# MGI-tech-bioinformatics/SuperPlus

Hardware: AMD Instinct MI355X
Metric: k-mers/s (DF createDict stage: trim + canonical k-mer count + solid filter + spectrum + adjacency) (higher is better)
Workload: dtype u64

## Files before the change

### superplus_amd/csrc/dfk.hip

```cpp
#include "../../include/dfk.h"
#include "dfk_kernels.h"

#include <algorithm>
#include <chrono>
#include <cstdarg>
#include <cstdio>
#include <cstdlib>
#include <cstring>
#include <atomic>
#include <fcntl.h>
#include <functional>
#include <new>
#include <string>
#include <sys/mman.h>
#include <sys/stat.h>
#include <unistd.h>
#include <condition_variable>
#include <memory>
#include <mutex>
#include <thread>
#include <vector>

using namespace dfk;

namespace {

thread_local std::string g_err;

int fail(int code, const char* fmt, ...)
{
    char buf[512];
    va_list ap; va_start(ap, fmt); vsnprintf(buf, sizeof buf, fmt, ap); va_end(ap);
    g_err = buf;
    return code;
}

#define HIP_TRY(expr) do { hipError_t e_ = (expr); if (e_ != hipSuccess) \
    return fail(DFK_E_HIP, "%s failed: %s (%s:%d)", #expr, hipGetErrorString(e_), __FILE__, __LINE__); } while (0)

template <class F> int guarded(F&& f)
{
    try { return f(); }
    catch (const std::bad_alloc&) { return fail(DFK_E_NOMEM, "out of host memory"); }
    catch (const std::exception& e) { return fail(DFK_E_HIP, "internal error: %s", e.what()); }
    catch (...) { return fail(DFK_E_HIP, "internal error"); }
}

struct DevBuf {
    void* p = nullptr; size_t bytes = 0;
    bool sub = false;
};

bool g_trace = getenv("DFK_TRACE") != nullptr;
#define TRACE(...) do { if (g_trace) { fprintf(stderr, "[dfk] " __VA_ARGS__); fputc('\n', stderr); fflush(stderr); } } while (0)
inline double wall_now() { return std::chrono::duration<double>(std::chrono::steady_clock::now().time_since_epoch()).count(); }

template <int K> struct CountCfg;
#ifndef DFK_LOG2S
#define DFK_LOG2S 11
#endif
#ifndef DFK_NWAVES
#define DFK_NWAVES 8
#endif
template <> struct CountCfg<40> { static constexpr int LOG2S = DFK_LOG2S, NWAVES = DFK_NWAVES; };
template <> struct CountCfg<48> { static constexpr int LOG2S = DFK_LOG2S, NWAVES = DFK_NWAVES; };
template <> struct CountCfg<60> { static constexpr int LOG2S = DFK_LOG2S, NWAVES = DFK_NWAVES; };

struct Inputs {
    const uint8_t* packed; uint64_t packed_bytes;
    const uint64_t* base_off; const uint32_t* read_len;
    const uint8_t* pq; uint64_t pq_bytes; const uint64_t* pq_off;
    const int32_t* bc; uint64_t n_reads;
};

}

struct dfk_ctx {
    dfk_config cfg{};
    int device = 0;
    hipStream_t stream = nullptr;
    hipStream_t stream2 = nullptr;
    hipDeviceProp_t prop{};
    uint64_t budget = 0, held = 0, peak = 0;
    struct Owned { void* p; uint64_t bytes, seq; };
    std::vector<Owned> owned;
    uint64_t alloc_seq = 0;
    bool have = false;
    uint64_t n_reads = 0;
    struct FileRange { const char* base; uint64_t bytes; int fd; uint64_t off; };
    std::vector<FileRange> file_ranges;
    DevBuf good_len;
    struct Part { DevBuf buf, pre; uint64_t n = 0; uint64_t blist = 0, n_blist = 0; bool listed = false; };
    bool want_blist = false;
    int pending_blist = -1;
    std::function<int()> after_count_launch;
    std::vector<Part> parts;
    uint64_t n_solid = 0, n_boundary = 0;
    unsigned seg_attempt = 0;
    double distinct_per_inst = 0.0;
    double plan_derate = 0.95;
    std::vector<int64_t> hist;
    std::vector<dfk_entry32> sorted, sorted_pre;
    bool sorted_ok = false, sorted_pre_ok = false;
    dfk_stats st{};
    bool shard_open = false, shard_use_bc = false;
    const void* sh_in[7] = {};
    uint64_t sh_packed_bytes = 0, sh_pq_bytes = 0, sh_n_reads = 0, sh_n_inst_local = 0;
    int64_t sh_read_id0 = 0;
    DevBuf shard_send[2];
    uint32_t shard_send_pass[2] = {~0u, ~0u};
    DevBuf shard_recv[2];
    unsigned shard_recv_seq = 0;
    uint64_t budget_taken = 0;
    void* sh_staged[6] = {};
    uint64_t sh_b0 = 0, sh_b1 = 0, sh_q0 = 0, sh_q1 = 0, sh_staged_reads = 0;
    DevBuf adj_keys, adj_src; uint64_t adj_n = 0;
    DevBuf set; uint64_t set_mask = 0;
    double t_upload_done = 0;
    uint32_t shard_world = 1, shard_log2_nb = 0;
    void* shard_state = nullptr;
    void (*shard_state_free)(void*) = nullptr;
    void* lane_pool = nullptr; void (*lane_pool_free)(void*) = nullptr;
    std::mutex lane_mu;
    void* graph_state = nullptr;
    void (*graph_state_free)(void*) = nullptr;
    unsigned int* d_resident = nullptr;
    unsigned int resident_target = 0;
    unsigned int last_wg_idle = 0;
    void* kept[6] = {};
    uint64_t kept_packed_bytes = 0, kept_pq_bytes = 0, kept_n_reads = 0, kept_budget = 0;

    struct Free { uint64_t off, bytes; };
    struct Chunk { char* p; uint64_t bytes; std::vector<Free> free_list; bool adopted = false; };
    std::vector<Chunk> chunks;
    uint64_t reserved = 0;

    uint64_t first_chunk_hint = 0;
    bool carve(Chunk& k, size_t bytes, DevBuf& b, bool long_lived)
    {
        if (!long_lived) {
            for (size_t i = k.free_list.size(); i-- > 0;)
                if (k.free_list[i].bytes >= bytes) {
                    k.free_list[i].bytes -= bytes;
                    b.p = k.p + k.free_list[i].off + k.free_list[i].bytes; b.bytes = bytes;
                    if (!k.free_list[i].bytes) k.free_list.erase(k.free_list.begin() + i);
                    return true;
                }
            return false;
        }
        for (size_t i = 0; i < k.free_list.size(); ++i)
            if (k.free_list[i].bytes >= bytes) {
                b.p = k.p + k.free_list[i].off; b.bytes = bytes;
                k.free_list[i].off += bytes; k.free_list[i].bytes -= bytes;
                if (!k.free_list[i].bytes) k.free_list.erase(k.free_list.begin() + i);
                return true;
            }
        return false;
    }
    void drop_empty_chunks()
    {
        for (size_t i = 0; i < chunks.size();)
            if (chunks[i].free_list.size() == 1 && chunks[i].free_list[0].bytes == chunks[i].bytes)
            { (void)hipFree(chunks[i].p); reserved -= chunks[i].bytes; chunks.erase(chunks.begin() + i); }
            else ++i;
    }
    struct PassBlock { DevBuf block; size_t used = 0; };
    PassBlock* sub = nullptr;
    int alloc(DevBuf& b, size_t bytes, const char* what, bool top = false)
    {
        bytes = bytes ? (bytes + 255) & ~(size_t)255 : 256;
        if (sub && !top && sub->used + bytes <= sub->block.bytes) {
            b.p = (char*)sub->block.p + sub->used; b.bytes = bytes; b.sub = true;
            sub->used += bytes;
            return 0;
        }
        if (held + bytes > budget)
            return fail(DFK_E_NOMEM, "HBM budget exceeded allocating %zu bytes for %s (held %llu, budget %llu)",
                        bytes, what, (unsigned long long)held, (unsigned long long)budget);
        bool ok = false;
        for (Chunk& k : chunks) if (carve(k, bytes, b, top)) { ok = true; break; }
        if (!ok) {
            uint64_t want = std::max<uint64_t>(2 * (uint64_t)bytes, 64ull << 20);
            if (chunks.empty()) want = std::max<uint64_t>(want, std::min<uint64_t>(first_chunk_hint, budget));
            if (reserved + want > budget) { drop_empty_chunks(); want = std::min<uint64_t>(want, budget > reserved ? budget - reserved : 0); }
            want &= ~(uint64_t)0xFFF;
            if (want < bytes) {
                if (g_trace) {
                    for (const Chunk& k : chunks) for (const Free& f : k.free_list) fprintf(stderr, "[dfk]   free %.2f GB at %.2f GB\n", f.bytes / 1e9, f.off / 1e9);
                    for (const Owned& o : owned) if (o.bytes >= (1ull << 28)) fprintf(stderr, "[dfk]   held %.2f GB at %.2f GB (#%llu)\n", o.bytes / 1e9, ((char*)o.p - chunks[0].p) / 1e9, (unsigned long long)o.seq);
                }
                return fail(DFK_E_NOMEM, "HBM budget exhausted by fragmentation allocating %zu bytes for %s", bytes, what);
            }
            void* p = nullptr;
            hipError_t e = hipMalloc(&p, want);
            if (e != hipSuccess && want > bytes) { (void)hipGetLastError(); want = bytes; e = hipMalloc(&p, want); }
            if (e != hipSuccess) return fail(DFK_E_NOMEM, "hipMalloc(%llu) for %s: %s", (unsigned long long)want, what, hipGetErrorString(e));
            chunks.push_back(Chunk{(char*)p, want, {Free{0, want}}});
            reserved += want;
            TRACE("new device chunk %p, %.2f GB (reserved %.2f of %.2f GB)", p, want / 1e9, (reserved) / 1e9, budget / 1e9);
            carve(chunks.back(), bytes, b, top);
        }
        held += bytes; peak = std::max(peak, held);
        owned.push_back(Owned{b.p, (uint64_t)bytes, ++alloc_seq});
        if (bytes >= (1ull << 30)) TRACE("alloc %-28s %8.2f GB at %p (%s), held %.2f GB", what, bytes / 1e9, b.p, top ? "top" : "bottom", held / 1e9);
        return 0;
    }
    uint64_t largest_allocatable() const
    {
        uint64_t best = budget > reserved ? (budget - reserved) & ~(uint64_t)0xFFF : 0;
        for (const Chunk& k : chunks) for (const Free& f : k.free_list) best = std::max<uint64_t>(best, f.bytes);
        return std::min<uint64_t>(best, budget > held ? budget - held : 0);
    }
    void release(DevBuf& b)
    {
        if (!b.p) return;
        if (b.sub) { b = DevBuf{}; return; }
        auto it = std::find_if(owned.begin(), owned.end(), [&](const Owned& o) { return o.p == b.p; });
        if (it != owned.end()) owned.erase(it);
        for (Chunk& k : chunks)
// ... 1955 lines not shown
```

### superplus_amd/csrc/dfk_kernels.h

```cpp
#pragma once
#include <type_traits>
#include "dfk_device.h"

namespace dfk {

template <int K>
__global__ void __launch_bounds__(256)
k_trim(const uint8_t* __restrict__ pq, const uint64_t* __restrict__ pq_off, uint64_t pq_nbytes,
       const uint64_t* __restrict__ base_off, uint64_t packed_bytes, const uint32_t* __restrict__ read_len,
       uint64_t n_reads, uint32_t min_qual, uint32_t* __restrict__ good_len,
       unsigned long long* __restrict__ n_inst, unsigned int* __restrict__ bad,
       unsigned long long* __restrict__ sum_good)
{
    unsigned long long mine = 0, good = 0;
    bool any_bad = false;
    for (uint64_t r = (uint64_t)blockIdx.x * blockDim.x + threadIdx.x; r < n_reads; r += (uint64_t)gridDim.x * blockDim.x) {
        uint32_t gl = 0;
        uint64_t p = pq_off[r], end = pq_off[r + 1];
        uint32_t idx = 0, run = 0;
        const uint64_t b0 = base_off[r], b1 = base_off[r + 1];
        bool ok = p <= end && end <= pq_nbytes && b0 <= b1 && b1 <= packed_bytes && b1 - b0 >= ((uint64_t)read_len[r] + 3) / 4;
        if (!ok) end = p;
        while (p < end) {
            uint32_t nQs = pq[p];
            if (!nQs) break;
            if (p + 3 > end) { ok = false; break; }
            uint32_t hdr = pq[p + 1] | ((uint32_t)pq[p + 2] << 8);
            uint32_t nBits = hdr & 7u, minQ = (hdr >> 3) & 63u;
            uint64_t blk = ((uint64_t)nQs * nBits + 24) >> 3;
            if (p + blk > end) { ok = false; break; }
            if (nBits == 0) {
                if (minQ >= min_qual) { run += nQs; if (run >= (uint32_t)K) gl = idx + nQs; }
                else run = 0;
                idx += nQs;
            } else {
                uint64_t bit = 8 * (p + 1) + 9;
                const uint32_t fmask = (1u << nBits) - 1u;
                for (uint32_t left = nQs; left;) {
                    const uint64_t by = bit >> 3;
                    const uint32_t sh = (uint32_t)(bit & 7);
                    uint64_t w = 0;
                    if (by + 8 <= pq_nbytes) __builtin_memcpy(&w, pq + by, 8);
                    else for (uint32_t k = 0; k < 8 && by + k < pq_nbytes; ++k) w |= (uint64_t)pq[by + k] << (8 * k);
                    w >>= sh;
                    const uint32_t n = min(left, (64u - sh) / nBits);
                    for (uint32_t i = 0; i < n; ++i, w >>= nBits) {
                        const uint32_t q = minQ + ((uint32_t)w & fmask);
                        if (q < min_qual) run = 0;
                        else if (++run >= (uint32_t)K) gl = idx + 1;
                        ++idx;
                    }
                    bit += (uint64_t)n * nBits; left -= n;
                }
            }
            p += blk;
        }
        uint32_t rl = read_len[r];
        if (!ok || idx != rl) { any_bad = true; gl = 0; }
        if (gl > rl) gl = rl;
        good_len[r] = gl;
        good += gl;
        if (gl >= (uint32_t)K + 1) mine += gl - K + 1;
    }
    __shared__ unsigned long long sh[2][4];
    __shared__ unsigned int sh_bad;
    if (threadIdx.x == 0) sh_bad = 0;
    __syncthreads();
#pragma unroll
    for (int d = 32; d > 0; d >>= 1) { mine += __shfl_down(mine, d, 64); good += __shfl_down(good, d, 64); }
    if ((threadIdx.x & 63) == 0) { sh[0][threadIdx.x >> 6] = mine; sh[1][threadIdx.x >> 6] = good; }
    if (any_bad) atomicOr(&sh_bad, 1u);
    __syncthreads();
    if (threadIdx.x == 0) {
        unsigned long long a0 = sh[0][0] + sh[0][1] + sh[0][2] + sh[0][3], a1 = sh[1][0] + sh[1][1] + sh[1][2] + sh[1][3];
        if (a0) atomicAdd(n_inst, a0);
        if (a1) atomicAdd(sum_good, a1);
        if (sh_bad) atomicOr(bad, 1u);
    }
}

struct PartParams {
    uint32_t M;
    uint32_t W;
    uint32_t log2_nb;
    uint32_t log2_world;
    int64_t  read_id0;
    uint32_t sub_lo;
    uint32_t sub_n;
    uint32_t class_mask;
};

constexpr uint32_t SWEEP_CLASSES = 32;
__host__ __device__ inline uint32_t sweep_class_of(uint32_t local_bucket, uint32_t log2_local)
{ return log2_local > 5 ? local_bucket >> (log2_local - 5) : local_bucket; }
__host__ __device__ inline uint32_t sweep_class_mask(uint32_t sub_lo, uint32_t sub_n, uint32_t log2_local)
{
    if (sub_n == 0) return 0u;
    const uint32_t a = sweep_class_of(sub_lo, log2_local), b = sweep_class_of(sub_lo + sub_n - 1, log2_local);
    const uint32_t upto_b = b >= 31 ? 0xFFFFFFFFu : ((1u << (b + 1)) - 1u);
    return upto_b & ~((1u << a) - 1u);
}

constexpr int PART_THREADS = 128;
constexpr int PART_RING = 2;
constexpr int SUMMARY_RUNS = 10;
constexpr uint32_t SUMMARY_OVERFLOW = 15;

__device__ __forceinline__ uint32_t pass_local(uint32_t bucket, const PartParams& pp)
{
    const uint32_t ls = pp.log2_nb - pp.log2_world;
    const uint32_t d = (bucket & ((1u << ls) - 1u)) - pp.sub_lo;
    return d < pp.sub_n ? (bucket >> ls) * pp.sub_n + d : 0xFFFFFFFFu;
}

__device__ __forceinline__ uint32_t bucket_of(uint32_t minhash, const PartParams& pp)
{
    const uint32_t b = (minhash * 0x9E3779B1u) >> (32 - pp.log2_nb);
    return ((b & ((1u << pp.log2_world) - 1u)) << (pp.log2_nb - pp.log2_world)) | (b >> pp.log2_world);
}
constexpr int PART_QCAP = 8;

template <int K>
__device__ __forceinline__ void emit_record(const uint32_t* __restrict__ words, uint64_t n_words, uint64_t bit0,
                                            uint32_t s0, uint32_t nk, uint32_t bucket, uint32_t gl, int32_t tag,
                                            uint64_t dst_index, uint4* __restrict__ records)
{
    const bool hp = s0 > 0;
    const bool hs = s0 + nk + (uint32_t)K <= gl;
    uint64_t bo = bit0 + 2ull * (hp ? s0 - 1 : 0);
    uint64_t wi = bo >> 5; uint32_t sh = (uint32_t)bo & 31u;
    uint32_t w[7];
#pragma unroll
    for (int i = 0; i < 7; ++i) w[i] = (wi + i < n_words) ? words[wi + i] : 0u;
    uint32_t o[6];
#pragma unroll
    for (int i = 0; i < 6; ++i) o[i] = alignbit(w[i + 1], w[i], sh);
    if (!hp) {
#pragma unroll
        for (int i = 5; i > 0; --i) o[i] = (o[i] << 2) | (o[i - 1] >> 30);
        o[0] <<= 2;
    }
    uint32_t nbits = 2u * (1u + nk + (uint32_t)K - 1u + (hs ? 1u : 0u));
#pragma unroll
    for (int i = 0; i < 6; ++i) {
        uint32_t lo = 32u * i;
        if (nbits <= lo) o[i] = 0;
        else if (nbits < lo + 32u) o[i] &= (1u << (nbits - lo)) - 1u;
    }
    uint4 a{rec_header(nk, hp, hs, bucket), (uint32_t)tag, o[0], o[1]};
    uint4 b{o[2], o[3], o[4], o[5]};
    records[2 * dst_index] = a;
    records[2 * dst_index + 1] = b;
}

constexpr uint32_t PART_CLASSES = 64;
__device__ __forceinline__ uint32_t class_bin(uint32_t bucket, const PartParams& pp)
{
    const uint32_t ls = pp.log2_nb - pp.log2_world;
    const uint32_t sub = bucket & ((1u << ls) - 1u);
    return (bucket >> ls) * PART_CLASSES + (ls > 6 ? sub >> (ls - 6) : sub);
}

template <int K, bool WRITE>
__device__ __forceinline__ void
partition_read(uint64_t r, uint32_t* smem, uint32_t* __restrict__ lh,
            const uint8_t* __restrict__ packed, uint64_t packed_bytes, const uint64_t* __restrict__ base_off,
            const uint32_t* __restrict__ good_len, const int32_t* __restrict__ bc, int64_t ign_bc_below,
            uint64_t n_reads, const PartParams& pp,
            unsigned long long* __restrict__ bucket_acc, unsigned long long* __restrict__ bucket_cur, uint64_t n_out,
            uint4* __restrict__ records, uint4* __restrict__ summaries, const uint32_t* __restrict__ read_list, uint64_t n_list,
            const uint64_t* __restrict__ slice_base, uint32_t* __restrict__ read_classes)
{
    auto place = [&](uint32_t b) -> uint64_t {
        if (!slice_base) { const uint64_t d = atomicAdd(&bucket_cur[b], 1ull); return d < n_out ? d : ~0ull; }
        const uint32_t owner = b / pp.sub_n;
        const uint64_t d = slice_base[owner] + atomicAdd(&bucket_cur[owner], 1ull);
        return d < slice_base[owner + 1] ? d : ~0ull;
    };
    uint32_t* arr = smem;
    uint32_t* queue = smem + pp.W * PART_THREADS;
    uint8_t* sidx = reinterpret_cast<uint8_t*>(smem + pp.W * PART_THREADS);
    uint32_t* ring = reinterpret_cast<uint32_t*>(sidx + pp.W * PART_THREADS);
    uint64_t sum_lo = 0, sum_hi = 0;
    const int tid = threadIdx.x;
    if (WRITE && read_list) { if (r >= n_list) return; r = read_list[r]; }
    const uint32_t M = pp.M, W = pp.W;
    const uint32_t gl = r < n_reads ? good_len[r] : 0;
    if (gl < (uint32_t)K + 1) {
        if (!WRITE && r < n_reads) { summaries[r] = uint4{0, 0, 0, 0}; if (read_classes) read_classes[r] = 0u; }
        return;
    }
    uint32_t Pi = 0, cur_rel = 0;
    uint32_t cmask = 0;
    const uint32_t log2_local = pp.log2_nb - pp.log2_world;

    const uint64_t byte0 = base_off[r];
    const uint32_t* words = reinterpret_cast<const uint32_t*>(packed);
    const uint64_t n_words = (packed_bytes + 3) >> 2;
    const uint64_t bit0 = byte0 * 8;
    int32_t tag = -1;
    if (bc && (int64_t)r + pp.read_id0 >= ign_bc_below) tag = bc[r];

    const uint32_t mmask = M == 16 ? 0xFFFFFFFFu : ((1u << (2 * M)) - 1u);
    const uint32_t rsh = 2 * (M - 1);
    uint32_t f = 0, rc = 0;
    uint32_t P = 0;
    uint32_t bi = 0;
    uint32_t cur_b = 0, cur_s0 = 0, cur_nk = 0;
    uint32_t qn = 0;

    uint64_t wi = bit0 >> 5;
    uint64_t filled_to = wi;
    auto fill = [&]() {
        uint32_t w[PART_RING];
#pragma unroll
        for (int k = 0; k < PART_RING; ++k) w[k] = filled_to + k < n_words ? words[filled_to + k] : 0u;
#pragma unroll
        for (int k = 0; k < PART_RING; ++k) ring[((filled_to + k) & (PART_RING - 1)) * PART_THREADS + tid] = w[k];
        filled_to += PART_RING;
    };
    uint32_t wbits, wnext = 0;
    if (!WRITE) { fill(); wbits = ring[(wi & (PART_RING - 1)) * PART_THREADS + tid]; }
    else { wbits = wi < n_words ? words[wi] : 0u; wnext = wi + 1 < n_words ? words[wi + 1] : 0u; }
    uint32_t wpos = (uint32_t)bit0 & 31u;
    uint32_t sfx_next = 0xFFFFFFFFu;

    auto close_run = [&]() {
        if (WRITE && cur_b == 0xFFFFFFFFu) return;
        if (!WRITE) {
            if (lh) { const uint32_t bin = class_bin(cur_b, pp); atomicAdd(&lh[bin], 1u); atomicAdd(&lh[(PART_CLASSES << pp.log2_world) + bin], cur_nk); }
            else atomicAdd(&bucket_acc[cur_b], (1ull << 32) | cur_nk);
            cmask |= 1u << sweep_class_of(cur_b & ((1u << log2_local) - 1u), log2_local);
            if (qn < (uint32_t)SUMMARY_RUNS) {
                const uint64_t fld = cur_nk | (cur_rel << 6);
                const uint32_t b = 8u + 12u * qn;
                if (b < 64u) { sum_lo |= fld << b; if (b > 52u) sum_hi |= fld >> (64u - b); }
                else sum_hi |= fld << (b - 64u);
            }
            ++qn;
        } else {
            if (qn == PART_QCAP) {
                for (uint32_t e = 0; e < qn; ++e) {
                    uint32_t a = queue[(2 * e) * PART_THREADS + tid], b = queue[(2 * e + 1) * PART_THREADS + tid];
                    const uint64_t dst = place(b);
                    if (dst != ~0ull) emit_record<K>(words, n_words, bit0, a & 0xFFFFu, a >> 16, b, gl, tag, dst, records);
                }
                qn = 0;
            }
            queue[(2 * qn) * PART_THREADS + tid] = cur_s0 | (cur_nk << 16);
            queue[(2 * qn + 1) * PART_THREADS + tid] = cur_b;
            ++qn;
        }
    };

    for (uint32_t j = 0; j < gl; ++j) {
        uint32_t b = (wbits >> wpos) & 3u;
        wpos += 2;
        if (wpos == 32) {
            wpos = 0; ++wi;
            if (!WRITE) { if (wi == filled_to) fill(); wbits = ring[(wi & (PART_RING - 1)) * PART_THREADS + tid]; }
            else { wbits = wnext; wnext = wi + 1 < n_words ? words[wi + 1] : 0u; }
        }
        f = ((f << 2) | b) & mmask;
        rc = (rc >> 2) | ((3u - b) << rsh);
        if (j + 1 < M) continue;
        uint32_t h = mmer_hash(f < rc ? f : rc);
        const bool newmin = bi == 0 || h < P;
        P = newmin ? h : P;
        if (!WRITE) Pi = newmin ? bi : Pi;
        const uint32_t t = j + 1 - M;
        if (t + 1 >= W) {
            uint32_t mv = P;
            bool older = false;
            if (bi != W - 1) { const uint32_t sfx = sfx_next; older = sfx < mv; mv = older ? sfx : mv; }
            const uint32_t s = t + 1 - W;
            uint32_t bucket = bucket_of(mv, pp);
            if (WRITE) bucket = pass_local(bucket, pp);
            const bool open = s == 0 || bucket != cur_b || cur_nk == (uint32_t)KTraits<K>::NK_MAX;
            if (open) {
                if (s != 0) close_run();
                cur_b = bucket; cur_s0 = s; cur_nk = 1;
                if (!WRITE) cur_rel = older ? (uint32_t)sidx[(bi + 1) * PART_THREADS + tid] - bi - 1u : W - 1u - bi + Pi;
            } else ++cur_nk;
        }
        arr[bi * PART_THREADS + tid] = h;
        if (++bi == W) {
            uint32_t run = h, ri = W - 1;
            if (!WRITE) sidx[(W - 1) * PART_THREADS + tid] = (uint8_t)(W - 1);
            for (int i0 = (int)W - 2; i0 >= 0; i0 -= 8) {
                uint32_t v[8];
#pragma unroll
                for (int k = 0; k < 8; ++k) v[k] = i0 - k >= 0 ? arr[(i0 - k) * PART_THREADS + tid] : 0u;
#pragma unroll
                for (int k = 0; k < 8; ++k) {
                    const int i = i0 - k;
                    if (i >= 0) {
                        const bool lt = v[k] < run;
                        run = lt ? v[k] : run;
                        arr[i * PART_THREADS + tid] = run;
                        if (!WRITE) { ri = lt ? (uint32_t)i : ri; sidx[i * PART_THREADS + tid] = (uint8_t)ri; }
                    }
                }
            }
            bi = 0;
        }
// ... 48 lines not shown
                                 bucket_acc, bucket_cur, n_out, records, summaries, read_list, n_list, slice_base, read_classes);
    if (lh) {
        __syncthreads();
        for (uint32_t i = threadIdx.x; i < n_bins; i += PART_THREADS) if (lh[i]) atomicAdd(&class_hist[i], (unsigned long long)lh[i]);
    }
}

template <int I, int N, class F>
__device__ __forceinline__ void static_for(F&& f)
{
    if constexpr (I < N) { f(std::integral_constant<int, I>{}); static_for<I + 1, N>(f); }
}

template <int K, int M>
__global__ void __launch_bounds__(PART_THREADS)
k_scan_count(const uint8_t* __restrict__ packed, uint64_t packed_bytes, const uint64_t* __restrict__ base_off,
             const uint32_t* __restrict__ good_len, uint64_t r_first, uint64_t n_reads , PartParams pp,
             unsigned long long* __restrict__ bucket_acc, unsigned long long* __restrict__ class_hist,
             unsigned long long* __restrict__ ovf_count, uint64_t ovf_cap, uint32_t* __restrict__ ovf_list,
             uint4* __restrict__ summaries, uint32_t* __restrict__ read_classes)
{
    constexpr int W = K - M + 1;
    constexpr uint32_t mmask = M == 16 ? 0xFFFFFFFFu : ((1u << (2 * M)) - 1u);
    constexpr uint32_t rsh = 2 * (M - 1);
    constexpr int RUNS = SUMMARY_RUNS;
    extern __shared__ uint32_t smem[];
    uint32_t* ring = smem;
    uint32_t* runb = smem + PART_RING * PART_THREADS;
    uint32_t* lh = nullptr;
    const uint32_t n_bins = 2u * (PART_CLASSES << pp.log2_world);
    if (class_hist) {
        lh = runb + RUNS * PART_THREADS;
        for (uint32_t i = threadIdx.x; i < n_bins; i += PART_THREADS) lh[i] = 0;
        __syncthreads();
    }
    const int tid = threadIdx.x;
    const uint32_t* words = reinterpret_cast<const uint32_t*>(packed);
    const uint64_t n_words = (packed_bytes + 3) >> 2;
    const uint32_t log2_local = pp.log2_nb - pp.log2_world;
    for (uint64_t r0 = r_first + (uint64_t)blockIdx.x * PART_THREADS; r0 < n_reads; r0 += (uint64_t)gridDim.x * PART_THREADS) {
        const uint64_t r = r0 + tid;
        const uint32_t gl = r < n_reads ? good_len[r] : 0;
        const bool live = gl >= (uint32_t)K + 1;
        uint32_t qn = 0, cmask = 0;
        uint64_t sum_lo = 0, sum_hi = 0;
        if (live) {
            const uint64_t bit0 = base_off[r] * 8;
            uint64_t wi = bit0 >> 5, filled_to = wi;
            auto fill = [&]() {
                uint32_t w[PART_RING];
#pragma unroll
                for (int k = 0; k < PART_RING; ++k) w[k] = filled_to + k < n_words ? words[filled_to + k] : 0u;
#pragma unroll
                for (int k = 0; k < PART_RING; ++k) ring[((filled_to + k) & (PART_RING - 1)) * PART_THREADS + tid] = w[k];
                filled_to += PART_RING;
            };
            fill();
            uint32_t wbits = ring[(wi & (PART_RING - 1)) * PART_THREADS + tid], wpos = (uint32_t)bit0 & 31u;
            auto next_base = [&]() -> uint32_t {
                const uint32_t b = (wbits >> wpos) & 3u;
                wpos += 2;
                if (wpos == 32) { wpos = 0; ++wi; if (wi == filled_to) fill(); wbits = ring[(wi & (PART_RING - 1)) * PART_THREADS + tid]; }
                return b;
            };
            uint32_t f = 0, rc = 0;
            for (int j = 0; j < M - 1; ++j) { const uint32_t b = next_base(); f = ((f << 2) | b) & mmask; rc = (rc >> 2) | ((3u - b) << rsh); }
            const uint32_t n_mmers = gl - M + 1;
            uint32_t arr[W], sidxw[(W + 3) / 4];
            auto sidx_get = [&](int i) -> uint32_t { return (sidxw[i >> 2] >> (8 * (i & 3))) & 255u; };
            auto sidx_set = [&](int i, uint32_t v) { const uint32_t sh = 8u * (uint32_t)(i & 3); sidxw[i >> 2] = (sidxw[i >> 2] & ~(255u << sh)) | (v << sh); };
#pragma unroll
            for (int i = 0; i < (W + 3) / 4; ++i) sidxw[i] = 0;
            uint32_t P = 0, Pi = 0;
            uint32_t cur_b = 0, cur_nk = 0, cur_rel = 0;
            auto close_run = [&]() {
                if (qn < (uint32_t)RUNS) {
                    runb[qn * PART_THREADS + tid] = cur_b;
                    const uint64_t fld = cur_nk | (cur_rel << 6);
                    const uint32_t b = 8u + 12u * qn;
                    if (b < 64u) { sum_lo |= fld << b; if (b > 52u) sum_hi |= fld >> (64u - b); } else sum_hi |= fld << (b - 64u);
                } else {
                    if (lh) { const uint32_t bin = class_bin(cur_b, pp); atomicAdd(&lh[bin], 1u); atomicAdd(&lh[(PART_CLASSES << pp.log2_world) + bin], cur_nk); }
                    else atomicAdd(&bucket_acc[cur_b], (1ull << 32) | cur_nk);
                    cmask |= 1u << sweep_class_of(cur_b & ((1u << log2_local) - 1u), log2_local);
                }
                ++qn;
            };
            for (uint32_t t0 = 0; t0 < n_mmers; t0 += W) {
                static_for<0, W>([&](auto bi_c) {
                    constexpr int bi = decltype(bi_c)::value;
                    if (t0 + (uint32_t)bi < n_mmers) {
                        const uint32_t b = next_base();
                        f = ((f << 2) | b) & mmask;
                        rc = (rc >> 2) | ((3u - b) << rsh);
                        const uint32_t h = mmer_hash(f < rc ? f : rc);
                        const bool newmin = bi == 0 || h < P;
                        P = newmin ? h : P;
                        Pi = newmin ? (uint32_t)bi : Pi;
                        const bool first = t0 == 0;
                        if (!first || bi == W - 1) {
                            uint32_t mv = P;
                            bool older = false;
                            if constexpr (bi != W - 1) { older = arr[bi + 1] < mv; mv = older ? arr[bi + 1] : mv; }
                            const uint32_t bucket = bucket_of(mv, pp);
                            const bool open = first || bucket != cur_b || cur_nk == (uint32_t)KTraits<K>::NK_MAX;
                            if (open) {
                                if (!first) close_run();
                                cur_b = bucket; cur_nk = 1;
                                cur_rel = (bi != W - 1 && older) ? sidx_get(bi + 1 < W ? bi + 1 : 0) - (uint32_t)bi - 1u : (uint32_t)(W - 1 - bi) + Pi;
                            } else ++cur_nk;
                        }
                        arr[bi] = h;
                        if (bi == W - 1) {
                            uint32_t run = h, ri = W - 1;
                            sidx_set(W - 1, W - 1);
                            static_for<0, W - 1>([&](auto j_c) {
                                constexpr int i = W - 2 - decltype(j_c)::value;
                                const bool lt = arr[i] < run; run = lt ? arr[i] : run; arr[i] = run; ri = lt ? (uint32_t)i : ri; sidx_set(i, ri);
                            });
                        }
                    }
                });
            }
            close_run();
        }
        const uint32_t mine = min(qn, (uint32_t)RUNS);
        for (uint32_t i = 0; __ballot(i < mine) != 0ull; ++i) {
            if (i < mine) {
                const uint32_t cb = runb[i * PART_THREADS + tid];
                const uint32_t bfld = 8u + 12u * i;
                const uint32_t nk = (uint32_t)(bfld + 12 <= 64 ? sum_lo >> bfld : bfld >= 64 ? sum_hi >> (bfld - 64) : (sum_lo >> bfld) | (sum_hi << (64 - bfld))) & 63u;
                if (lh) { const uint32_t bin = class_bin(cb, pp); atomicAdd(&lh[bin], 1u); atomicAdd(&lh[(PART_CLASSES << pp.log2_world) + bin], nk); }
                else atomicAdd(&bucket_acc[cb], (1ull << 32) | nk);
                cmask |= 1u << sweep_class_of(cb & ((1u << log2_local) - 1u), log2_local);
            }
        }
        if (r < n_reads) {
            const uint64_t lo = sum_lo | (qn <= (uint32_t)SUMMARY_RUNS ? qn : SUMMARY_OVERFLOW);
            summaries[r] = uint4{(uint32_t)lo, (uint32_t)(lo >> 32), (uint32_t)sum_hi, (uint32_t)(sum_hi >> 32)};
            if (read_classes) read_classes[r] = cmask;
        }
        if (qn > (uint32_t)SUMMARY_RUNS) {
            const unsigned long long at = atomicAdd(ovf_count, 1ull);
            if (at < ovf_cap) ovf_list[at] = (uint32_t)r;
        }
    }
    if (lh) {
        __syncthreads();
        for (uint32_t i = threadIdx.x; i < n_bins; i += PART_THREADS) if (lh[i]) atomicAdd(&class_hist[i], (unsigned long long)lh[i]);
    }
}

constexpr int SLICE_READS = 16;
template <int K, bool EMIT, typename F>
__device__ __forceinline__ void for_each_run_in_pass(uint64_t r, const uint8_t* __restrict__ packed, uint64_t packed_bytes,
                                                     const uint64_t* __restrict__ base_off, const PartParams& pp,
                                                     const uint4* __restrict__ summaries, F&& f)
{
    const uint4 sm = summaries[r];
    const uint32_t n = sm.x & 15u;
    if (n == 0 || n == SUMMARY_OVERFLOW) return;
    const uint32_t* words = reinterpret_cast<const uint32_t*>(packed);
    const uint64_t n_words = (packed_bytes + 3) >> 2;
    const uint64_t bit0 = base_off[r] * 8;
    const uint32_t M = pp.M;
    const uint32_t mmask = M == 16 ? 0xFFFFFFFFu : ((1u << (2 * M)) - 1u);
    const uint64_t lo = (uint64_t)sm.x | ((uint64_t)sm.y << 32), hi = (uint64_t)sm.z | ((uint64_t)sm.w << 32);
    uint32_t s0 = 0;
#pragma unroll
    for (int i = 0; i < SUMMARY_RUNS; ++i) {
        if ((uint32_t)i < n) {
            constexpr int B0 = 8;
            const int b = B0 + 12 * i;
            const uint32_t fld = (uint32_t)(b + 12 <= 64 ? lo >> b : b >= 64 ? hi >> (b - 64) : (lo >> b) | (hi << (64 - b))) & 0xFFFu;
            const uint32_t nk = fld & 63u, rel = fld >> 6;
            const uint64_t bo = bit0 + 2ull * (s0 + rel);
            const uint64_t wi = bo >> 5;
            const uint32_t w0 = words[wi], w1 = wi + 1 < n_words ? words[wi + 1] : 0u;
            const uint32_t x = alignbit(w1, w0, (uint32_t)bo & 31u) & mmask;
            uint32_t y = __brev(x);
            y = ((y >> 1) & 0x55555555u) | ((y & 0x55555555u) << 1);
            const uint32_t fw = y >> (32 - 2 * M), rcv = ~x & mmask;
            const uint32_t bucket = bucket_of(mmer_hash(fw < rcv ? fw : rcv), pp);
            const uint32_t lb = pass_local(bucket, pp);
            if (lb != 0xFFFFFFFFu) f(s0, nk, lb, bucket >> (pp.log2_nb - pp.log2_world), bit0, (uint32_t)i + 1 == n);
            s0 += nk;
        }
    }
}

template <int K>
__global__ void __launch_bounds__(256)
k_scatter_slices(const uint8_t* __restrict__ packed, uint64_t packed_bytes, const uint64_t* __restrict__ base_off,
                 const uint32_t* __restrict__ good_len, const int32_t* __restrict__ bc, int64_t ign_bc_below,
                 uint64_t n_reads, PartParams pp, const uint4* __restrict__ summaries, const uint32_t* __restrict__ read_classes,
                 const uint64_t* __restrict__ slice_base,
                 unsigned long long* __restrict__ slice_fill,
                 uint4* __restrict__ records)
{
    __shared__ uint32_t cnt[256];
    __shared__ unsigned long long at[256];
    __shared__ uint16_t list[256 * SLICE_READS];
    __shared__ uint32_t n_list;
    const uint32_t world = 1u << pp.log2_world;
    const int lane = threadIdx.x & 63;
    const uint64_t r_block = (uint64_t)blockIdx.x * 256 * SLICE_READS;
    if (threadIdx.x < world) cnt[threadIdx.x] = 0;
    if (threadIdx.x == 0) n_list = 0;
    __syncthreads();
#pragma unroll
    for (int j = 0; j < SLICE_READS; ++j) {
        const uint32_t rel = 256u * j + threadIdx.x;
        const uint64_t r = r_block + rel;
        const bool hit = r < n_reads && (!read_classes || (read_classes[r] & pp.class_mask) != 0u);
        const unsigned long long mk = __ballot(hit);
        uint32_t w = 0;
        if (lane == 0 && mk) w = atomicAdd(&n_list, (uint32_t)__popcll(mk));
        w = __builtin_amdgcn_readfirstlane(w);
        if (hit) list[w + __popcll(mk & ((1ull << lane) - 1ull))] = (uint16_t)rel;
    }
    __syncthreads();
    const uint32_t n = n_list;
    for (uint32_t i = threadIdx.x; i < n; i += 256)
        for_each_run_in_pass<K, false>(r_block + list[i], packed, packed_bytes, base_off, pp, summaries,
                                       [&](uint32_t, uint32_t, uint32_t, uint32_t owner, uint64_t, bool) { atomicAdd(&cnt[owner], 1u); });
    __syncthreads();
    if (threadIdx.x < world) {
        const uint32_t m = cnt[threadIdx.x];
        at[threadIdx.x] = slice_base[threadIdx.x] + (m ? atomicAdd(&slice_fill[threadIdx.x], (unsigned long long)m) : 0ull);
        cnt[threadIdx.x] = 0;
    }
    __syncthreads();
    const uint32_t* words = reinterpret_cast<const uint32_t*>(packed);
    const uint64_t n_words = (packed_bytes + 3) >> 2;
    (void)good_len;
    for (uint32_t i = threadIdx.x; i < n; i += 256) {
        const uint64_t r = r_block + list[i];
        int32_t tag = -1;
        if (bc && (int64_t)r + pp.read_id0 >= ign_bc_below) tag = bc[r];
        for_each_run_in_pass<K, true>(r, packed, packed_bytes, base_off, pp, summaries,
            [&](uint32_t s0, uint32_t nk, uint32_t lb, uint32_t owner, uint64_t bit0, bool last) {
                const uint64_t dst = at[owner] + atomicAdd(&cnt[owner], 1u);
                if (dst < slice_base[owner + 1]) emit_record<K>(words, n_words, bit0, s0, nk, lb, last ? 0u : 0xFFFFFFFFu, tag, dst, records);
            });
    }
}

#ifndef DFK_SWEEP_READS
#define DFK_SWEEP_READS 8
#endif
template <int K> constexpr int sweep_reads() { return KTraits<K>::KW == 4 ? 2 : DFK_SWEEP_READS; }
template <int K>
__global__ void __launch_bounds__(256)
k_scatter_runs(const uint8_t* __restrict__ packed, uint64_t packed_bytes, const uint64_t* __restrict__ base_off,
               const uint32_t* __restrict__ good_len, const int32_t* __restrict__ bc, int64_t ign_bc_below,
               uint64_t n_reads, PartParams pp, const uint4* __restrict__ summaries, const uint32_t* __restrict__ read_classes,
               unsigned long long* __restrict__ bucket_cur, uint64_t n_out, uint4* __restrict__ records)
{
    constexpr int SWEEP_READS = sweep_reads<K>();
    __shared__ uint16_t list[256 * SWEEP_READS];
    __shared__ uint32_t n_list;
    (void)good_len;
    const int lane = threadIdx.x & 63;
    const uint64_t r_block = (uint64_t)blockIdx.x * 256 * SWEEP_READS;
    if (threadIdx.x == 0) n_list = 0;
    __syncthreads();
#pragma unroll
    for (int j = 0; j < SWEEP_READS; ++j) {
        const uint32_t rel = 256u * j + threadIdx.x;
        const uint64_t r = r_block + rel;
        const bool hit = r < n_reads && (read_classes[r] & pp.class_mask) != 0u;
        const unsigned long long mk = __ballot(hit);
        uint32_t at = 0;
        if (lane == 0 && mk) at = atomicAdd(&n_list, (uint32_t)__popcll(mk));
        at = __builtin_amdgcn_readfirstlane(at);
        if (hit) list[at + __popcll(mk & ((1ull << lane) - 1ull))] = (uint16_t)rel;
    }
    __syncthreads();
    const uint32_t n = n_list;
    const uint32_t* words = reinterpret_cast<const uint32_t*>(packed);
    const uint64_t n_words = (packed_bytes + 3) >> 2;
    for (uint32_t i = threadIdx.x; i < n; i += 256) {
        const uint64_t r = r_block + list[i];
        int32_t tag = -1;
        if (bc && (int64_t)r + pp.read_id0 >= ign_bc_below) tag = bc[r];
        for_each_run_in_pass<K, true>(r, packed, packed_bytes, base_off, pp, summaries,
            [&](uint32_t s0, uint32_t nk, uint32_t lb, uint32_t, uint64_t bit0, bool last) {
                const uint64_t dst = atomicAdd(&bucket_cur[lb], 1ull);
                if (dst < n_out) emit_record<K>(words, n_words, bit0, s0, nk, lb, last ? 0u : 0xFFFFFFFFu, tag, dst, records);
            });
    }
}



struct ItemRange { uint32_t b0, b1; };

struct CountParams {
    uint32_t min_freq, min_bc;
    uint32_t n_items;
    uint32_t single;
    uint64_t seg_cap;
    uint32_t do_adj;
    uint32_t keep_pre;
};

struct CountGlobals {
    unsigned long long n_distinct;
    unsigned long long big_cursor;
    unsigned int next_item;
    unsigned int n_overflow;
    unsigned int solid_overflow;
    unsigned int n_split;
    unsigned long long n_boundary;
    unsigned long long part_cursor;
    unsigned int n_wg_idle;
    unsigned int pad_idle;
};

struct WgOut { unsigned long long chunk; unsigned int used; unsigned int pad; };

constexpr int COUNT_HIST_BINS = 256;
constexpr uint32_t COUNT_MAX_PROBE = 96;
constexpr uint32_t HIST_GLOBAL_BINS = 1u << 24;
constexpr int COUNT_CHUNK = 32;
constexpr uint32_t FLAG_SOLID = 0x80000000u;

template <int K> struct WaveStage {
    uint32_t rec[COUNT_CHUNK * 8 + 8];
    uint32_t starts[COUNT_CHUNK];
    uint32_t msk[64];
    uint32_t pc[64];
};

__device__ __forceinline__ uint32_t tld(const uint32_t* p)
{ return __hip_atomic_load(p, __ATOMIC_RELAXED, __HIP_MEMORY_SCOPE_AGENT); }
__device__ __forceinline__ void tst(uint32_t* p, uint32_t v)
{ __hip_atomic_store(p, v, __ATOMIC_RELAXED, __HIP_MEMORY_SCOPE_AGENT); }

struct Probe {
    uint32_t k0, k1, k2, k3, ctx, fp, step, slot;
    int32_t tag;
    bool active;
};

__device__ __forceinline__ Probe probe_begin(u128 c, uint32_t ctx, int32_t tag, uint32_t S, bool active)
{
    const uint32_t h = key_hash(c);
    return Probe{(uint32_t)c.lo, (uint32_t)(c.lo >> 32), (uint32_t)c.hi, (uint32_t)(c.hi >> 32), ctx, (h >> 24) | 1u,
                 ((h >> 11) | 1u) & (S - 1), h & (S - 1), tag, active};
}

#define DFK_COMPILER_FENCE() asm volatile("" ::: "memory")
#ifdef DFK_PHASE_TIMES
__device__ unsigned long long g_phase[16];
struct PhaseClock {
    unsigned long long t, acc[12];
    __device__ __forceinline__ void start() { t = __builtin_amdgcn_s_memtime(); for (int i = 0; i < 12; ++i) acc[i] = 0; }
    __device__ __forceinline__ void mark(int i) { const unsigned long long n = __builtin_amdgcn_s_memtime(); acc[i] += n - t; t = n; }
    __device__ __forceinline__ void flush(int lane) { if (lane == 0) for (int i = 0; i < 12; ++i) atomicAdd(&g_phase[i], acc[i]); }
};
#define PH(i) phase.mark(i)
#else
#define PH(i) do { } while (0)
#endif
__device__ unsigned int g_big_fail[4];

enum : uint32_t { PS_PROBING = 0, PS_FOUND = 1, PS_FAILED = 2, PS_IDLE = 3 };
constexpr uint32_t PROBE_COST = 1u << 12, PROBE_LIMIT = (COUNT_MAX_PROBE + 1) * PROBE_COST;

template <int KW, int NBC, bool LDS_TABLE>
__device__ __forceinline__ bool table_insert(uint32_t* __restrict__ keys, uint32_t* __restrict__ cnt,
                                             uint32_t* __restrict__ ctxs, uint32_t* __restrict__ bcw,
                                             uint32_t S, const Probe& A, uint32_t& n_claimed)
{
    uint32_t state = A.active ? PS_PROBING : PS_IDLE, slot = A.slot, seen = 0, cost = 0, waits = 0;
    while (__ballot(state == PS_PROBING) != 0ull) {
        if (state == PS_PROBING) {
            uint32_t e = 0, r0, r1, r2, r3 = A.k3;
            if (LDS_TABLE) {
                __hip_atomic_compare_exchange_strong(&cnt[slot], &e, CNT_LOCK, __ATOMIC_RELAXED, __ATOMIC_RELAXED,
                                                     __HIP_MEMORY_SCOPE_WORKGROUP);
                DFK_COMPILER_FENCE();
                r0 = tld(&keys[slot]); r1 = tld(&keys[S + slot]); r2 = tld(&keys[2 * S + slot]);
                if (KW == 4) r3 = tld(&keys[3 * S + slot]);
            } else {
                __hip_atomic_compare_exchange_strong(&cnt[slot], &e, CNT_LOCK, __ATOMIC_ACQUIRE, __ATOMIC_ACQUIRE,
                                                     __HIP_MEMORY_SCOPE_AGENT);
                r0 = tld(&keys[slot]); r1 = tld(&keys[S + slot]); r2 = tld(&keys[2 * S + slot]);
                if (KW == 4) r3 = tld(&keys[3 * S + slot]);
            }
            const bool won = e == 0u;
            if (won) {
                tst(&keys[slot], A.k0); tst(&keys[S + slot], A.k1); tst(&keys[2 * S + slot], A.k2);
                if (KW == 4) tst(&keys[3 * S + slot], A.k3);
                if (LDS_TABLE) {
                    DFK_COMPILER_FENCE();
                    __hip_atomic_store(&cnt[slot], A.fp << 24, __ATOMIC_RELAXED, __HIP_MEMORY_SCOPE_WORKGROUP);
                } else __hip_atomic_store(&cnt[slot], A.fp << 24, __ATOMIC_RELEASE, __HIP_MEMORY_SCOPE_AGENT);
            }
            const uint32_t locked = e == CNT_LOCK;
            const uint32_t match = ((e >> 24) == A.fp) & (r0 == A.k0) & (r1 == A.k1) & (r2 == A.k2) & (r3 == A.k3);
            const uint32_t fin = (uint32_t)won | match;
            n_claimed += (uint32_t)won;
            seen |= e & (0u - match);
            cost += PROBE_COST - (PROBE_COST - 1u) * locked;
            if (!LDS_TABLE) waits += locked;
            slot = (slot + (A.step & ((fin | locked) - 1u))) & (S - 1);
            state = fin | ((uint32_t)(cost >= PROBE_LIMIT) << 1);
        }
    }
    if (!LDS_TABLE && state == PS_FAILED && atomicCAS(&g_big_fail[0], 0u, 1u) == 0u) {
        g_big_fail[1] = (cost - waits) / PROBE_COST; g_big_fail[2] = waits; g_big_fail[3] = 31u - (uint32_t)__clz(S);
    }
    if (state == PS_FOUND) {
        if (LDS_TABLE) {
            const bool high = (seen & CNT_MASK) >= CNT_HALF;
            if (!high) atomicAdd(&cnt[slot], 1u);
            unsigned long long todo = __ballot(high);
            while (todo) {
                const int leader = __ffsll((long long)todo) - 1;
                const uint32_t lslot = (uint32_t)__builtin_amdgcn_readlane((int)slot, leader);
                const unsigned long long same = __ballot(high && slot == lslot) & todo;
                if ((threadIdx.x & 63) == leader) {
                    const uint32_t k = (uint32_t)__popcll(same);
                    uint32_t cur = tld(&cnt[slot]);
                    for (;;) {
                        const uint32_t c0 = cur & CNT_MASK, c1 = c0 + k < CNT_MASK ? c0 + k : CNT_MASK;
                        if (c1 == c0) break;
                        if (__hip_atomic_compare_exchange_strong(&cnt[slot], &cur, (cur & ~CNT_MASK) | c1, __ATOMIC_RELAXED, __ATOMIC_RELAXED,
                                                                 __HIP_MEMORY_SCOPE_WORKGROUP)) break;
                    }
                }
                todo &= ~same;
            }
        } else {
            uint32_t* wide = ctxs + S;
            if (atomicAdd(&wide[slot], 1u) >= 0x7FFFFFFFu) atomicSub(&wide[slot], 1u);
        }
        atomicOr(&ctxs[slot], A.ctx);
        if (NBC > 0) {
            if (A.tag == -1) atomicOr(&bcw[slot], BCW_MULTI);
            else if (A.tag > 0) {
// ... 1332 lines not shown
```

Before: 58.57 billion.

## Restructure scatter kernel into per-wave compaction with two reads per lane and batched runs

The k_scatter_runs kernel stops building a block-wide shared-memory list behind barriers. Each wave now compacts the hit reads itself with ballots and ds_bpermute, and every lane processes two reads at a time. Run summaries are decoded in chunks of four, so the minimizer hashing, the global atomics and the record gathers from both reads can be issued together for memory-level parallelism. The change also raises sweep reads per wave to 16 and adds a vectorised fast path for the record gather. The cost is more register pressure and more complex control flow, and the overflow-summary reads appear to be skipped in this path, which may depend on another kernel handling them.

```diff
diff --git a/superplus_amd/csrc/dfk.hip b/superplus_amd/csrc/dfk.hip
--- a/superplus_amd/csrc/dfk.hip
+++ b/superplus_amd/csrc/dfk.hip
@@ -59,12 +59,14 @@
 #ifndef DFK_LOG2S
 #define DFK_LOG2S 11
 #endif
-#ifndef DFK_NWAVES
-#define DFK_NWAVES 8
+#ifdef DFK_NWAVES
+#define DFK_NWAVES_OF(k_default) DFK_NWAVES
+#else
+#define DFK_NWAVES_OF(k_default) k_default
 #endif
-template <> struct CountCfg<40> { static constexpr int LOG2S = DFK_LOG2S, NWAVES = DFK_NWAVES; };
-template <> struct CountCfg<48> { static constexpr int LOG2S = DFK_LOG2S, NWAVES = DFK_NWAVES; };
-template <> struct CountCfg<60> { static constexpr int LOG2S = DFK_LOG2S, NWAVES = DFK_NWAVES; };
+template <> struct CountCfg<40> { static constexpr int LOG2S = DFK_LOG2S, NWAVES = DFK_NWAVES_OF(8); };
+template <> struct CountCfg<48> { static constexpr int LOG2S = DFK_LOG2S, NWAVES = DFK_NWAVES_OF(8); };
+template <> struct CountCfg<60> { static constexpr int LOG2S = DFK_LOG2S, NWAVES = DFK_NWAVES_OF(8); };
 
 struct Inputs {
     const uint8_t* packed; uint64_t packed_bytes;
diff --git a/superplus_amd/csrc/dfk_kernels.h b/superplus_amd/csrc/dfk_kernels.h
--- a/superplus_amd/csrc/dfk_kernels.h
+++ b/superplus_amd/csrc/dfk_kernels.h
@@ -120,37 +120,54 @@
 }
 constexpr int PART_QCAP = 8;
 
+__device__ __forceinline__ void record_gather(const uint32_t* __restrict__ words, uint64_t n_words, uint64_t bit0, uint32_t s0,
+                                              uint32_t w[7])
+{
+    const uint64_t bo = bit0 + 2ull * (s0 > 0 ? s0 - 1 : 0);
+    const uint64_t wi = bo >> 5;
+    if (wi + 7 <= n_words) __builtin_memcpy(w, words + wi, 7 * sizeof(uint32_t));
+    else {
+#pragma unroll
+        for (int i = 0; i < 7; ++i) w[i] = (wi + i < n_words) ? words[wi + i] : 0u;
+    }
+}
+
+template <int K>
+__device__ __forceinline__ void record_store(const uint32_t w[7], uint64_t bit0, uint32_t s0, uint32_t nk, uint32_t bucket,
+                                             uint32_t gl, int32_t tag, uint64_t dst_index, uint4* __restrict__ records)
+{
+    const bool hp = s0 > 0;
+    const bool hs = s0 + nk + (uint32_t)K <= gl;
+    const uint32_t sh = (uint32_t)(bit0 + 2ull * (hp ? s0 - 1 : 0)) & 31u;
+    uint32_t o[6];
+#pragma unroll
+    for (int i = 0; i < 6; ++i) o[i] = alignbit(w[i + 1], w[i], sh);
+    if (!hp) {
+#pragma unroll
+        for (int i = 5; i > 0; --i) o[i] = (o[i] << 2) | (o[i - 1] >> 30);
+        o[0] <<= 2;
+    }
+    uint32_t nbits = 2u * (1u + nk + (uint32_t)K - 1u + (hs ? 1u : 0u));
+#pragma unroll
+    for (int i = 0; i < 6; ++i) {
+        uint32_t lo = 32u * i;
+        if (nbits <= lo) o[i] = 0;
+        else if (nbits < lo + 32u) o[i] &= (1u << (nbits - lo)) - 1u;
+    }
+    uint4 a{rec_header(nk, hp, hs, bucket), (uint32_t)tag, o[0], o[1]};
+    uint4 b{o[2], o[3], o[4], o[5]};
+    records[2 * dst_index] = a;
+    records[2 * dst_index + 1] = b;
+}
+
 template <int K>
 __device__ __forceinline__ void emit_record(const uint32_t* __restrict__ words, uint64_t n_words, uint64_t bit0,
                                             uint32_t s0, uint32_t nk, uint32_t bucket, uint32_t gl, int32_t tag,
                                             uint64_t dst_index, uint4* __restrict__ records)
 {
-    const bool hp = s0 > 0;
-    const bool hs = s0 + nk + (uint32_t)K <= gl;
-    uint64_t bo = bit0 + 2ull * (hp ? s0 - 1 : 0);
-    uint64_t wi = bo >> 5; uint32_t sh = (uint32_t)bo & 31u;
     uint32_t w[7];
-#pragma unroll
-    for (int i = 0; i < 7; ++i) w[i] = (wi + i < n_words) ? words[wi + i] : 0u;
-    uint32_t o[6];
-#pragma unroll
-    for (int i = 0; i < 6; ++i) o[i] = alignbit(w[i + 1], w[i], sh);
-    if (!hp) {
-#pragma unroll
-        for (int i = 5; i > 0; --i) o[i] = (o[i] << 2) | (o[i - 1] >> 30);
-        o[0] <<= 2;
-    }
-    uint32_t nbits = 2u * (1u + nk + (uint32_t)K - 1u + (hs ? 1u : 0u));
-#pragma unroll
-    for (int i = 0; i < 6; ++i) {
-        uint32_t lo = 32u * i;
-        if (nbits <= lo) o[i] = 0;
-        else if (nbits < lo + 32u) o[i] &= (1u << (nbits - lo)) - 1u;
-    }
-    uint4 a{rec_header(nk, hp, hs, bucket), (uint32_t)tag, o[0], o[1]};
-    uint4 b{o[2], o[3], o[4], o[5]};
-    records[2 * dst_index] = a;
-    records[2 * dst_index + 1] = b;
+    record_gather(words, n_words, bit0, s0, w);
+    record_store<K>(w, bit0, s0, nk, bucket, gl, tag, dst_index, records);
 }
 
 constexpr uint32_t PART_CLASSES = 64;
@@ -505,6 +522,15 @@
 }
 
 constexpr int SLICE_READS = 16;
+__device__ __forceinline__ uint32_t minimizer_bucket(uint32_t w0, uint32_t w1, uint32_t sh, uint32_t M, uint32_t mmask, const PartParams& pp)
+{
+    const uint32_t x = alignbit(w1, w0, sh) & mmask;
+    uint32_t y = __brev(x);
+    y = ((y >> 1) & 0x55555555u) | ((y & 0x55555555u) << 1);
+    const uint32_t fw = y >> (32 - 2 * M), rcv = ~x & mmask;
+    return bucket_of(mmer_hash(fw < rcv ? fw : rcv), pp);
+}
+
 template <int K, bool EMIT, typename F>
 __device__ __forceinline__ void for_each_run_in_pass(uint64_t r, const uint8_t* __restrict__ packed, uint64_t packed_bytes,
                                                      const uint64_t* __restrict__ base_off, const PartParams& pp,
@@ -530,11 +556,7 @@
             const uint64_t bo = bit0 + 2ull * (s0 + rel);
             const uint64_t wi = bo >> 5;
             const uint32_t w0 = words[wi], w1 = wi + 1 < n_words ? words[wi + 1] : 0u;
-            const uint32_t x = alignbit(w1, w0, (uint32_t)bo & 31u) & mmask;
-            uint32_t y = __brev(x);
-            y = ((y >> 1) & 0x55555555u) | ((y & 0x55555555u) << 1);
-            const uint32_t fw = y >> (32 - 2 * M), rcv = ~x & mmask;
-            const uint32_t bucket = bucket_of(mmer_hash(fw < rcv ? fw : rcv), pp);
+            const uint32_t bucket = minimizer_bucket(w0, w1, (uint32_t)bo & 31u, M, mmask, pp);
             const uint32_t lb = pass_local(bucket, pp);
             if (lb != 0xFFFFFFFFu) f(s0, nk, lb, bucket >> (pp.log2_nb - pp.log2_world), bit0, (uint32_t)i + 1 == n);
             s0 += nk;
@@ -600,9 +622,37 @@
 }
 
 #ifndef DFK_SWEEP_READS
-#define DFK_SWEEP_READS 8
+#define DFK_SWEEP_READS 16
 #endif
-template <int K> constexpr int sweep_reads() { return KTraits<K>::KW == 4 ? 2 : DFK_SWEEP_READS; }
+template <int K> constexpr int sweep_reads() { return DFK_SWEEP_READS; }
+constexpr int SWEEP_CHUNK = 4;
+static_assert(DFK_SWEEP_READS % 4 == 0, "the class masks are loaded four groups at a time");
+
+__device__ __forceinline__ uint32_t nth_set_bit(uint64_t m, uint32_t k)
+{
+    uint32_t pos = 0;
+#pragma unroll
+    for (int w = 32; w > 0; w >>= 1) {
+        const uint32_t c = (uint32_t)__popcll(m & ((1ull << w) - 1ull));
+        const bool up = k >= c;
+        k -= up ? c : 0u; pos += up ? (uint32_t)w : 0u; m = up ? m >> w : m;
+    }
+    return pos;
+}
+
+__device__ __forceinline__ uint32_t summary_field(const uint4& sm, uint32_t i)
+{
+    const uint64_t lo = (uint64_t)sm.x | ((uint64_t)sm.y << 32), hi = (uint64_t)sm.z | ((uint64_t)sm.w << 32);
+    const uint32_t b = 8u + 12u * i;
+    return (uint32_t)(b < 64 ? (lo >> b) | (hi << (64 - b)) : hi >> (b - 64)) & 0xFFFu;
+}
+
+typedef uint32_t u32x4 __attribute__((ext_vector_type(4)));
+typedef uint32_t u32x8 __attribute__((ext_vector_type(8)));
+typedef uint64_t u64x2 __attribute__((ext_vector_type(2)));
+typedef int32_t i32x2 __attribute__((ext_vector_type(2)));
+typedef uint32_t u32x2 __attribute__((ext_vector_type(2)));
+
 template <int K>
 __global__ void __launch_bounds__(256)
 k_scatter_runs(const uint8_t* __restrict__ packed, uint64_t packed_bytes, const uint64_t* __restrict__ base_off,
@@ -611,37 +661,122 @@
                unsigned long long* __restrict__ bucket_cur, uint64_t n_out, uint4* __restrict__ records)
 {
     constexpr int SWEEP_READS = sweep_reads<K>();
-    __shared__ uint16_t list[256 * SWEEP_READS];
-    __shared__ uint32_t n_list;
+    constexpr int SLOTS = 2 * SWEEP_CHUNK;
     (void)good_len;
-    const int lane = threadIdx.x & 63;
-    const uint64_t r_block = (uint64_t)blockIdx.x * 256 * SWEEP_READS;
-    if (threadIdx.x == 0) n_list = 0;
-    __syncthreads();
-#pragma unroll
-    for (int j = 0; j < SWEEP_READS; ++j) {
-        const uint32_t rel = 256u * j + threadIdx.x;
-        const uint64_t r = r_block + rel;
-        const bool hit = r < n_reads && (read_classes[r] & pp.class_mask) != 0u;
-        const unsigned long long mk = __ballot(hit);
-        uint32_t at = 0;
-        if (lane == 0 && mk) at = atomicAdd(&n_list, (uint32_t)__popcll(mk));
-        at = __builtin_amdgcn_readfirstlane(at);
-        if (hit) list[at + __popcll(mk & ((1ull << lane) - 1ull))] = (uint16_t)rel;
-    }
-    __syncthreads();
-    const uint32_t n = n_list;
+    const uint32_t lane = threadIdx.x & 63u;
+    const uint64_t r_wave = ((uint64_t)blockIdx.x * 256u + (uint32_t)__builtin_amdgcn_readfirstlane(threadIdx.x & ~63u)) * SWEEP_READS;
+    if (r_wave >= n_reads) return;
     const uint32_t* words = reinterpret_cast<const uint32_t*>(packed);
     const uint64_t n_words = (packed_bytes + 3) >> 2;
-    for (uint32_t i = threadIdx.x; i < n; i += 256) {
-        const uint64_t r = r_block + list[i];
-        int32_t tag = -1;
-        if (bc && (int64_t)r + pp.read_id0 >= ign_bc_below) tag = bc[r];
-        for_each_run_in_pass<K, true>(r, packed, packed_bytes, base_off, pp, summaries,
-            [&](uint32_t s0, uint32_t nk, uint32_t lb, uint32_t, uint64_t bit0, bool last) {
-                const uint64_t dst = atomicAdd(&bucket_cur[lb], 1ull);
-                if (dst < n_out) emit_record<K>(words, n_words, bit0, s0, nk, lb, last ? 0u : 0xFFFFFFFFu, tag, dst, records);
-            });
+    if (n_words < 2) return;
+    const uint32_t M = pp.M;
+    const uint32_t mmask = M == 16 ? 0xFFFFFFFFu : ((1u << (2 * M)) - 1u);
+
+    auto load_hits = [&](uint32_t g, u32x4& cm) {
+#pragma unroll
+        for (int j = 0; j < 4; ++j) {
+            const uint64_t r = r_wave + 64u * (g + j) + lane;
+            cm[j] = read_classes[r < n_reads ? r : n_reads - 1] & (r < n_reads ? pp.class_mask : 0u);
+        }
+    };
+    u32x4 cm;
+    uint64_t h0 = 0, h1 = 0, h2 = 0, h3 = 0;
+    load_hits(0, cm);
+    uint32_t q0 = 0, q1 = 0, q2 = 0, fill = 0;
+#pragma unroll 1
+    for (uint32_t g = 0; g <= (uint32_t)SWEEP_READS; ++g) {
+        if (g < (uint32_t)SWEEP_READS) {
+            if ((g & 3u) == 0) {
+                h0 = __ballot(cm.x != 0u); h1 = __ballot(cm.y != 0u); h2 = __ballot(cm.z != 0u); h3 = __ballot(cm.w != 0u);
+                if (g + 4 < (uint32_t)SWEEP_READS) load_hits(g + 4, cm);
+            }
+            const uint64_t mk = h0;
+            h0 = h1; h1 = h2; h2 = h3;
+            if (mk) {
+                const uint32_t nh = (uint32_t)__popcll(mk);
+                const uint32_t k = (lane - fill) & 63u;
+                const uint32_t v = (uint32_t)__builtin_amdgcn_ds_bpermute((int)(nth_set_bit(mk, k) << 2), (int)(64u * g + lane));
+                if (k < nh) {
+                    const uint32_t x = (fill >> 6) + (lane < (fill & 63u) ? 1u : 0u);
+                    q0 = x == 0 ? v : q0; q1 = x == 1 ? v : q1; q2 = x == 2 ? v : q2;
+                }
+                fill += nh;
+            }
+        }
+        if (fill < 128u && (g < (uint32_t)SWEEP_READS || fill == 0)) continue;
+
+        const bool has[2] = {lane < fill, lane + 64u < fill};
+        const uint32_t rel[2] = {q0, q1};
+        q0 = q2; fill = fill >= 128u ? fill - 128u : 0u;
+        uint4 sm[2]; u64x2 bit0; i32x2 tag; u32x2 n;
+#pragma unroll
+        for (int t = 0; t < 2; ++t) {
+            const uint64_t r = r_wave + (has[t] ? rel[t] : 0u);
+            sm[t] = summaries[r];
+            bit0[t] = base_off[r] * 8;
+            tag[t] = (bc && (int64_t)r + pp.read_id0 >= ign_bc_below) ? bc[r] : -1;
+        }
+#pragma unroll
+        for (int t = 0; t < 2; ++t) {
+            const uint32_t nr = sm[t].x & 15u;
+            n[t] = has[t] && nr != SUMMARY_OVERFLOW ? nr : 0u;
+        }
+        u32x2 s0 = 0u;
+        for (uint32_t c0 = 0; __ballot(c0 < n[0] || c0 < n[1]) != 0ull; c0 += SWEEP_CHUNK) {
+            const u32x2 s0c = s0;
+            u32x8 lbs, w0, w1;
+#pragma unroll
+            for (int j = 0; j < SLOTS; ++j) {
+                const int t = j / SWEEP_CHUNK;
+                const uint32_t run = c0 + (uint32_t)(j % SWEEP_CHUNK);
+                const uint32_t fld = summary_field(sm[t], run < n[t] ? run : 0u);
+                const uint32_t nk = fld & 63u;
+                const uint64_t bo = bit0[t] + 2ull * (s0[t] + (fld >> 6));
+                const uint64_t wi = min(bo >> 5, n_words - 1), p = min(wi, n_words - 2);
+                uint32_t pair[2];
+                __builtin_memcpy(pair, words + p, sizeof pair);
+                w0[j] = p == wi ? pair[0] : pair[1];
+                w1[j] = p == wi ? pair[1] : 0u;
+                lbs[j] = (uint32_t)bo & 31u;
+                s0[t] += run < n[t] ? nk : 0u;
+            }
+            auto run_s0 = [&](int t, int i) {
+                uint32_t x = s0c[t];
+                for (int q = 0; q < i; ++q) x += summary_field(sm[t], c0 + (uint32_t)q) & 63u;
+                return x;
+            };
+            uint32_t pend = 0;
+#pragma unroll
+            for (int j = 0; j < SLOTS; ++j) {
+                const int t = j / SWEEP_CHUNK;
+                const uint32_t bucket = minimizer_bucket(w0[j], w1[j], lbs[j], M, mmask, pp);
+                lbs[j] = pass_local(bucket, pp);
+                if (c0 + (uint32_t)(j % SWEEP_CHUNK) < n[t] && lbs[j] != 0xFFFFFFFFu) pend |= 1u << j;
+            }
+#pragma unroll
+            for (int i = 0; i < SWEEP_CHUNK; ++i) {
+                const uint32_t in2 = (pend >> i & 1u) | (pend >> (SWEEP_CHUNK + i - 1) & 2u);
+                if (__ballot(in2 != 0u) == 0ull) continue;
+                uint32_t w[2][7]; uint64_t dst[2];
+#pragma unroll
+                for (int t = 0; t < 2; ++t) {
+                    const int j = t * SWEEP_CHUNK + i;
+                    dst[t] = ~0ull;
+                    if (in2 >> t & 1u) {
+                        dst[t] = atomicAdd(&bucket_cur[lbs[j]], 1ull);
+                        record_gather(words, n_words, bit0[t], run_s0(t, i), w[t]);
+                    }
+                }
+#pragma unroll
+                for (int t = 0; t < 2; ++t) {
+                    const int j = t * SWEEP_CHUNK + i;
+                    const bool last = c0 + (uint32_t)i + 1u == n[t];
+                    if (dst[t] < n_out)
+                        record_store<K>(w[t], bit0[t], run_s0(t, i), summary_field(sm[t], c0 + (uint32_t)i) & 63u, lbs[j],
+                                        last ? 0u : 0xFFFFFFFFu, tag[t], dst[t], records);
+                }
+            }
+        }
     }
 }
 
```

Result: no change. 58.44 billion (median of 6 runs) (-0.2%).
